# nicolaivicol/otto-recommender

Hardware: AMD Instinct MI355X
Metric: co-visit pairs/sec + candidates/sec at 220M events, 1/2/4/8 MI355X (higher is better)
Workload: dtype int32; 1 GPU; configs[1]: all 5 co-visitation rules, 220M events, 100k-session files; events=220000079, sessions=13435907, parallelism=files dealt over 1 GPU(s)

## Files before the change

### otto-recommender_amd/csrc/abi.hip

```cpp
#include <cstdarg>
#include <cstdlib>
#include <ctime>
#include <algorithm>
#include <mutex>
#include "prims.h"
#include "covis_kernels.h"
#include "table.h"

using namespace ottohip;

namespace ottohip {
static thread_local char g_err[1024] = "";
void set_error(const char* fmt, ...) {
  va_list ap;
  va_start(ap, fmt);
  vsnprintf(g_err, sizeof g_err, fmt, ap);
  va_end(ap);
}
}

namespace ottohip {
Ctx* ctx_base(ottohip_ctx* c) { return c; }

int ensure_part_stats(const ottohip_table* tc) {
// ... 566 lines not shown
  memset(&fo, 0, sizeof fo);
  if (fopts) OH_TRY(file_opts_setup(ctx, fopts, n_rules, R, fo, s));
  if (fo_parts) {
    fo = *fo_parts;
    OH_TRY(ctx->ws.get("fo_dropped", 1, &fo.dropped));
    OH_HIP(hipMemsetAsync(fo.dropped, 0, 8, s));
  }
  const bool FOon = fopts != nullptr || fo_parts != nullptr;
  const bool FOhist = FOon && !fo.cuts && !fo.parts && fo.hist != nullptr;
  const bool FOmir = FOon && fo.parts && fo.mirror_off != 0;
  const uint64_t n_slots = (fo_parts && fo_parts->mirror_off) ? 2 * P : P;
  if (ctx->spare.cap >= n_slots) {
    T->b = ctx->spare;
    ctx->spare = TableBufs();
  } else {
    const double t0 = alloc_log_begin();
    (void)hipDeviceSynchronize();
    ctx->spare.release();
    OH_TRY(T->b.alloc(n_slots));
    alloc_log_end(t0, "table", "slots", (size_t)n_slots * 17);
  }
  unsigned long long *stats, *lcount;
  OH_TRY(ws.get("stats", (size_t)STAT_STRIPES * STAT_STRIDE, &stats));
  OH_TRY(ws.get("lcount", 8, &lcount));
  hipMemsetAsync(stats, 0, (size_t)STAT_STRIPES * STAT_STRIDE * 8, s);
  hipMemsetAsync(err, 0, sizeof(int), s);
  if (getenv("OTTOHIP_REDUCE_DBG")) hipMemsetAsync(T->b.rule, 0xFF, n_slots, s);
  OutRows O;
  O.rule = T->b.rule; O.aid = T->b.aid; O.aid_next = T->b.aid_next; O.count = T->b.count; O.count_ge2 = T->b.count_ge2;
  O.cap = n_slots; O.stats = stats;
  T->sym_mask = R.sym_mask;
  static const int rdbg = getenv("OTTOHIP_REDUCE_DBG") ? atoi(getenv("OTTOHIP_REDUCE_DBG")) : 0;
  OutRows Osort = O;
  if (rdbg & 1) Osort.cap = 0;
  int herr = 0;

  static const int split_mean = getenv("OTTOHIP_SPLIT_MEAN") ? atoi(getenv("OTTOHIP_SPLIT_MEAN")) : SPLIT_MEAN;
  if (split_mean != SPLIT_MEAN) {
    const uint32_t v = (uint32_t)std::max(64, split_mean);
    OH_HIP(hipMemcpyToSymbolAsync(HIP_SYMBOL(c_split_mean), &v, sizeof v, 0, hipMemcpyHostToDevice, s));
    OH_HIP(hipStreamSynchronize(s));
  }
  static const char* runs_env = getenv("OTTOHIP_SPLIT_RUNS");
  if (runs_env && !strcmp(runs_env, "1")) {
    const uint32_t v = 1;
    OH_HIP(hipMemcpyToSymbolAsync(HIP_SYMBOL(c_split_runs), &v, sizeof v, 0, hipMemcpyHostToDevice, s));
    OH_HIP(hipStreamSynchronize(s));
// ... 10 lines not shown
    int8_t& st = lds_state[ctx->device & 63];
    if (st != (lds_leaf ? 2 : 1)) {
      const uint32_t on = lds_leaf ? 1u : 0u;
      OH_HIP(hipMemcpyToSymbolAsync(HIP_SYMBOL(c_lds_leaf), &on, sizeof on, 0, hipMemcpyHostToDevice, s));
      if (split_mean == SPLIT_MEAN) {
        const uint32_t v = lds_leaf ? (uint32_t)LDS_SPLIT_MEAN : (uint32_t)SPLIT_MEAN;
        OH_HIP(hipMemcpyToSymbolAsync(HIP_SYMBOL(c_split_mean), &v, sizeof v, 0, hipMemcpyHostToDevice, s));
      }
      OH_HIP(hipStreamSynchronize(s));
      st = lds_leaf ? 2 : 1;
    }
  }
  static const int hash_prio = getenv("OTTOHIP_HASH_PRIO") ? atoi(getenv("OTTOHIP_HASH_PRIO")) : 0;
  if (hash_prio) {
    const uint32_t v = (uint32_t)hash_prio;
    OH_HIP(hipMemcpyToSymbolAsync(HIP_SYMBOL(c_hash_prio), &v, sizeof v, 0, hipMemcpyHostToDevice, s));
    OH_HIP(hipStreamSynchronize(s));
  }
  int ph = ctx->begin("reduce", s, 4.0 * (double)P);
  uint64_t cap0 = (uint64_t)std::max<int64_t>(Rn, 1);
  TaskLists TL;
  TL.n = lcount;
  const uint64_t split_extra = P / 512 + 64;
  auto get_lists = [&](uint64_t capl, const char* split_name, int parity) -> int {
    static const char* names[2][N_SORT] = {{"t_sort0", "t_sort1", "t_sort2", "t_sort3", "t_sort4"},
                                           {"t_sort0b", "t_sort1b", "t_sort2b", "t_sort3b", "t_sort4b"}};
    for (int c = 0; c < N_SORT; ++c)
      if (int r = ws.get(names[parity][c], capl * sizeof(Task), reinterpret_cast<void**>(&TL.sort[c]))) return r;
    if (int r = ws.get(parity ? "t_hashb" : "t_hash", capl * sizeof(Task), reinterpret_cast<void**>(&TL.hash))) return r;
    if (int r = ws.get(parity ? "t_ldsb" : "t_lds", capl * sizeof(Task), reinterpret_cast<void**>(&TL.lds))) return r;
    if (int r = ws.get(split_name, (capl + split_extra) * sizeof(Task), reinterpret_cast<void**>(&TL.split))) return r;
    TL.cap = capl;
    return 0;
  };
  if ((rc = get_lists(cap0, "t_splitA", 0))) return rc;
  hipMemsetAsync(lcount, 0, 8 * 8, s);
  k_classify_rows<<<grid_for(Rn), 256, 0, s>>>(row_begin, Rn, P, Lt.WB, TL, err, row_base);
  const int agg_grid = ctx->n_cu * 8;
  static const bool overlap = !(getenv("OTTOHIP_REDUCE_OVERLAP") && !strcmp(getenv("OTTOHIP_REDUCE_OVERLAP"), "0"));
  hipStream_t s2 = nullptr;
  if (overlap) {
    OH_TRY(ctx->aux_stream());
    s2 = ctx->aux;
  }
  bool srcA = true;
  bool drained = false;
  const bool dbg = getenv("OTTOHIP_DEBUG") != nullptr;
  if (dbg) fprintf(stderr, "[ottohip] P=%llu rows=%lld\n", (unsigned long long)P, (long long)Rn);
  uint32_t* wcur0 = w0;
  const char* pipe_env = getenv("OTTOHIP_SPLIT_PIPE");
  const bool pipe = s2 != nullptr && !lds_leaf && !dbg && getenv("OTTOHIP_HASH_PROF") == nullptr &&
                    (pipe_env && atoi(pipe_env) == 1);
  const uint64_t PIPE_MIN_CHUNKS = getenv("OTTOHIP_SPLIT_PIPE_MIN") ? (uint64_t)atoll(getenv("OTTOHIP_SPLIT_PIPE_MIN")) : 2048;
  unsigned long long done[N_LISTS] = {};
  bool hash_early = false;
  auto launch_hash_range = [&](uint64_t lo, uint64_t hi, uint32_t* wb0, hipStream_t st) {
    if (hi <= lo) return;
    const int64_t nh = (int64_t)(hi - lo);
    const Task* th = TL.hash + lo;
    const unsigned hg = (unsigned)std::min<int64_t>(nh, (int64_t)agg_grid);
    if (FOhist)
      k_agg_hash<2><<<hg, AGG_T, 0, st>>>(th, nh, wb0, w1, row_key, R, Lt, n_rules, O, TL.split, lcount + N_SORT + 1, fo);
    else if (FOmir)
      k_agg_hash<3><<<hg, AGG_T, 0, st>>>(th, nh, wb0, w1, row_key, R, Lt, n_rules, O, TL.split, lcount + N_SORT + 1, fo);
    else if (FOon)
      k_agg_hash<1><<<hg, AGG_T, 0, st>>>(th, nh, wb0, w1, row_key, R, Lt, n_rules, O, TL.split, lcount + N_SORT + 1, fo);
    else
      k_agg_hash<<<hg, AGG_T, 0, st>>>(th, nh, wb0, w1, row_key, R, Lt, n_rules, O, TL.split, lcount + N_SORT + 1, fo);
  };
  auto launch_sorts = [&](const unsigned long long* lo, const unsigned long long* hi, uint32_t* wb0, hipStream_t st) {
    const unsigned sgrid = (unsigned)ctx->n_cu * 32;
#define OH_SORT(c, M)                                                                                          \
    if (hi[c] > lo[c]) {                                                                                       \
      const int64_t n_ = (int64_t)(hi[c] - lo[c]);                                                             \
      const Task* t_ = TL.sort[c] + lo[c];                                                                     \
      const unsigned g_ = (unsigned)std::min<uint64_t>(ceil_div(n_, 4), sgrid);                                \
      if (FOhist)                                                                                              \
        k_agg_sort<M, 2><<<g_, 256, (size_t)fo.nf * 8, st>>>(t_, n_, wb0, w1, row_key, R, Lt, n_rules, Osort, fo); \
      else if (FOmir)                                                                                          \
        k_agg_sort<M, 3><<<g_, 256, 0, st>>>(t_, n_, wb0, w1, row_key, R, Lt, n_rules, Osort, fo);             \
      else if (FOon)                                                                                           \
        k_agg_sort<M, 1><<<g_, 256, 0, st>>>(t_, n_, wb0, w1, row_key, R, Lt, n_rules, Osort, fo);             \
      else                                                                                                     \
        k_agg_sort<M><<<g_, 256, 0, st>>>(t_, n_, wb0, w1, row_key, R, Lt, n_rules, Osort, fo);                \
    }
    OH_SORT(0, 1) OH_SORT(1, 2) OH_SORT(2, 4) OH_SORT(3, 8) OH_SORT(4, 16)
#undef OH_SORT
  };
  for (int level = 0; level < 40; ++level) {
    wcur0 = (level == 0 || !w2) ? w0 : w2;
    unsigned long long nlist[N_LISTS];
    if ((rc = d2h(nlist, lcount, N_LISTS, s))) return rc;
    if ((rc = d2h(&herr, err, 1, s))) return rc;
    if (herr) { set_error("task list overflow / row too large (err=%d)", herr); return OTTOHIP_ELIMIT; }
    if (dbg) {
      fprintf(stderr, "[ottohip] level %d: sort %llu/%llu/%llu/%llu/%llu hash %llu split %llu lds %llu\n", level, nlist[0],
              nlist[1], nlist[2], nlist[3], nlist[4], nlist[N_SORT], nlist[N_SORT + 1], nlist[N_SORT + 2]);
      Task* lists[N_LISTS] = {TL.sort[0], TL.sort[1], TL.sort[2], TL.sort[3], TL.sort[4], TL.hash, TL.split, TL.lds};
      fprintf(stderr, "[ottohip] level %d words:", level);
      for (int c = 0; c < N_LISTS; ++c) {
        std::vector<Task> tv(nlist[c]);
        if (nlist[c]) (void)d2h(tv.data(), lists[c], nlist[c], s);
        unsigned long long sw = 0, mx = 0;
        for (auto& t : tv) { sw += t.len; mx = std::max<unsigned long long>(mx, t.len); }
        fprintf(stderr, " %llu(max %llu)", sw, mx);
        if (c == N_SORT + 1 && !tv.empty()) {
          unsigned long long hw[40] = {}, hn[40] = {};
          for (auto& t : tv) { const int b = 63 - __builtin_clzll((unsigned long long)t.len | 1ull); hw[b] += t.len; ++hn[b]; }
          fprintf(stderr, " [split by log2 len:");
          for (int b = 0; b < 40; ++b)
            if (hn[b]) fprintf(stderr, " 2^%d:%llu tasks/%llu words", b, hn[b], hw[b]);
          fprintf(stderr, "]");
        }
      }
      fprintf(stderr, "\n");
    }
    hipStream_t ss = s2 ? s2 : s;
    if (s2) { OH_HIP(hipEventRecord(ctx->ev_fork, s)); OH_HIP(hipStreamWaitEvent(s2, ctx->ev_fork, 0)); }
    static const bool hash_first = !(getenv("OTTOHIP_HASH_FIRST") && !strcmp(getenv("OTTOHIP_HASH_FIRST"), "0"));
    const bool hf = hash_first && nlist[N_SORT] > done[N_SORT];
    auto launch_hash = [&]() { launch_hash_range(done[N_SORT], nlist[N_SORT], wcur0, s); };
    if (hf) launch_hash();
    launch_sorts(done, nlist, wcur0, ss);
    if (s2) OH_HIP(hipEventRecord(ctx->ev_join[level & 1], s2));
    if (nlist[N_SORT + 2]) {
      const unsigned lg = (unsigned)std::min<uint64_t>(nlist[N_SORT + 2], (uint64_t)ctx->n_cu * 4);
      if (FOon)
        k_agg_lds<true><<<lg, LDS_T, 0, s>>>(TL.lds, (int64_t)nlist[N_SORT + 2], wcur0, w1, row_key, R, Lt, O, TL.split,
                                             lcount + N_SORT + 1, TL.cap + split_extra, err, fo);
      else
        k_agg_lds<<<lg, LDS_T, 0, s>>>(TL.lds, (int64_t)nlist[N_SORT + 2], wcur0, w1, row_key, R, Lt, O, TL.split,
                                       lcount + N_SORT + 1, TL.cap + split_extra, err, fo);
    }
    if (nlist[N_SORT] > done[N_SORT]) {
      static const bool hprof = getenv("OTTOHIP_HASH_PROF") != nullptr && !hash_first;
      if (hprof) {
        if ((rc = ws.get("hash_prof", (size_t)(2 * nlist[N_SORT]), &fo.prof))) return rc;
        OH_HIP(hipMemsetAsync(fo.prof, 0, 16 * nlist[N_SORT], s));
      }
      if (!hf) launch_hash();
      if (hprof) {
        std::vector<unsigned long long> pv(2 * nlist[N_SORT]);
        if ((rc = d2h(pv.data(), fo.prof, pv.size(), s))) return rc;
        std::vector<size_t> ord(nlist[N_SORT]);
// ... 32 lines not shown
        (rc = ws.get("sp_dgb", (size_t)ns + 1, &dgb)) || (rc = ws.get("sp_mtb", (size_t)ns + 1, &mtb)) ||
        (rc = ws.get("sp_tot", 6, &tot2)))
      return rc;
    k_split_prepare<<<grid_for(ns), 256, 0, s>>>(cur_split, ns, nch, ndg, nen);
    if ((rc = exclusive_scan_u32(ctx, nch, chb, ns, tot2, s)) || (rc = exclusive_scan_u32(ctx, ndg, dgb, ns, tot2 + 1, s)) ||
        (rc = exclusive_scan_u32(ctx, nen, mtb, ns, tot2 + 2, s)))
      return rc;
    if (pipe) k_split_half<<<1, 64, 0, s>>>(chb, dgb, ns, tot2, tot2 + 3);
    uint64_t tt[6] = {0, 0, 0, 0, 0, 0};
    if ((rc = d2h(tt, tot2, pipe ? 6 : 3, s))) return rc;
    const int64_t nchunks = (int64_t)tt[0], ndig = (int64_t)tt[1], nent = (int64_t)tt[2];
    const bool piped = pipe && (uint64_t)nchunks >= PIPE_MIN_CHUNKS && tt[3] > 0 && (int64_t)tt[3] < ns &&
                       tt[4] > 0 && (int64_t)tt[4] < nchunks && tt[5] > 0 && (int64_t)tt[5] < ndig;
    const uint32_t cA = piped ? (uint32_t)tt[4] : (uint32_t)nchunks;
    const int64_t dA = piped ? (int64_t)tt[5] : ndig;
    uint32_t *hmat, *ctask;
    uint64_t* hoff;
    if ((rc = ws.get("sp_hmat", (size_t)nent, &hmat)) || (rc = ws.get("sp_hoff", (size_t)nent + 1, &hoff)) ||
        (rc = ws.get("sp_ctask", (size_t)nchunks, &ctask)))
      return rc;
    k_split_chunk_task<<<grid_for(ns), 256, 0, s>>>(chb, nch, ns, ctask);
    k_split_hist<<<(unsigned)nchunks, SPLIT_T, 0, s>>>(cur_split, ns, chb, ctask, mtb, wcur0, w1, Lt.F, hmat);
    if ((rc = exclusive_scan_u32(ctx, hmat, hoff, nent, hoff + nent, s))) return rc;
    static const int sub = getenv("OTTOHIP_SPLIT_SUB") ? atoi(getenv("OTTOHIP_SPLIT_SUB")) : 4096;
    const char* lds_env = getenv("OTTOHIP_SPLIT_LDS");
    const bool split_lds = lds_env ? atoi(lds_env) != 0 : SPLIT_LDS_DEFAULT;
    const char* ldsmin_env = getenv("OTTOHIP_SPLIT_LDS_MIN");
    const uint32_t lds_min = (uint32_t)std::min(SPLIT_CH + 1, std::max(0, ldsmin_env ? atoi(ldsmin_env) : SPLIT_LDS_MIN));
    const int lds_t = getenv("OTTOHIP_SPLIT_LDS_T") ? atoi(getenv("OTTOHIP_SPLIT_LDS_T")) : SPLIT_LT;
    auto scatter = [&](uint32_t c0, uint32_t c1) {
      if (c1 <= c0) return;
      uint32_t max_len = SPLIT_CH;
      if (split_lds) {
        if (lds_t == 512)
          k_split_scatter_lds<512><<<c1 - c0, 512, 0, s>>>(cur_split, ns, chb, ctask, mtb, hoff, wcur0, w1, Lt.F, hmat, c0, lds_min);
        else
          k_split_scatter_lds<SPLIT_LT><<<c1 - c0, SPLIT_LT, 0, s>>>(cur_split, ns, chb, ctask, mtb, hoff, wcur0, w1, Lt.F, hmat, c0, lds_min);
        if (lds_min <= 1) return;
        max_len = lds_min - 1;
      }
      if (sub == 8192)
        k_split_scatter<8192><<<c1 - c0, SPLIT_T, 0, s>>>(cur_split, ns, chb, ctask, mtb, hoff, wcur0, w1, Lt.F, hmat, c0, max_len);
      else
        k_split_scatter<4096><<<c1 - c0, SPLIT_T, 0, s>>>(cur_split, ns, chb, ctask, mtb, hoff, wcur0, w1, Lt.F, hmat, c0, max_len);
    };
    scatter(0, cA);
    if (s2 && level >= 1) OH_HIP(hipStreamWaitEvent(s, ctx->ev_join[(level + 1) & 1], 0));
    const uint64_t capn = (uint64_t)ndig;
    if ((rc = get_lists(std::max(cap0, capn), srcA ? "t_splitB" : "t_splitA", (level + 1) & 1))) return rc;
    hipMemsetAsync(lcount, 0, 8 * 8, s);
    k_split_classify<<<grid_for(dA), 256, 0, s>>>(cur_split, ns, dgb, mtb, hoff, dA, TL, err, hmat, 0);
    if (piped) {
      if (getenv("OTTOHIP_SPLIT_PIPE_LOG")) fprintf(stderr, "[ottohip] level %d split pipelined at chunk %u of %lld\n", level, cA, (long long)nchunks);
      OH_HIP(hipEventRecord(ctx->ev_half, s));
      scatter(cA, (uint32_t)nchunks);
      if (ndig > dA)
        k_split_classify<<<grid_for(ndig - dA), 256, 0, s>>>(cur_split, ns, dgb, mtb, hoff, ndig, TL, err, hmat, dA);
      OH_HIP(hipStreamWaitEvent(ctx->aux2, ctx->ev_half, 0));
      unsigned long long nA[N_LISTS];
      if ((rc = d2h(nA, lcount, N_LISTS, ctx->aux2))) return rc;
      OH_HIP(hipStreamWaitEvent(s2, ctx->ev_half, 0));
      uint32_t* wb0 = w2 ? w2 : w0;
      if (nA[N_SORT]) {
        launch_hash_range(0, nA[N_SORT], wb0, s2);
        OH_HIP(hipEventRecord(ctx->ev_hash, s2));
        hash_early = true;
      }
      const unsigned long long zero[N_LISTS] = {};
      launch_sorts(zero, nA, wb0, s2);
      for (int c = 0; c <= N_SORT; ++c) done[c] = nA[c];
    }
    srcA = !srcA;
    if (hipGetLastError() != hipSuccess) { set_error("split launch failed"); return OTTOHIP_EHIP; }
  }
  ctx->end(ph, s);
  if (!drained) { set_error("reduce: split levels did not converge"); return OTTOHIP_ELIMIT; }
  std::vector<unsigned long long> stv((size_t)STAT_STRIPES * STAT_STRIDE);
  if ((rc = d2h(stv.data(), stats, stv.size(), s))) return rc;
  unsigned long long st[STAT_STRIDE] = {};
  for (int k = 0; k < STAT_STRIPES; ++k)
    for (int j = 0; j < STAT_STRIDE; ++j) st[j] += stv[(size_t)k * STAT_STRIDE + j];
  if (hipGetLastError() != hipSuccess) { set_error("reduce failed"); return OTTOHIP_EHIP; }
  unsigned long long U = 0, dropped = 0;
  for (int r = 0; r < n_rules; ++r) U += st[r * 4 + 0];
  const unsigned long long sum_pairs = st[STAT_RAW + 1], raw_rows = st[STAT_RAW];
  if (FOon) {
    if ((rc = d2h(&dropped, fo.dropped, 1, s))) return rc;
// ... 37 lines not shown
  if (hipHostMalloc(reinterpret_cast<void**>(&c->pinned), 64 * sizeof(uint64_t)) != hipSuccess) c->pinned = nullptr;
  *out = c;
  return 0;
}

void ottohip_ctx_destroy(ottohip_ctx* ctx) {
  if (!ctx) return;
  hipSetDevice(ctx->device);
  hipDeviceSynchronize();
  ctx->ws.release();
  ctx->spare.release();
  dev_trim();
  if (ctx->aux) {
    hipStreamDestroy(ctx->aux);
    if (ctx->aux2) hipStreamDestroy(ctx->aux2);
    if (ctx->ev_half) hipEventDestroy(ctx->ev_half);
    if (ctx->ev_hash) hipEventDestroy(ctx->ev_hash);
    hipEventDestroy(ctx->ev_fork);
    hipEventDestroy(ctx->ev_join[0]);
    hipEventDestroy(ctx->ev_join[1]);
  }
  for (auto e : ctx->event_pool) hipEventDestroy(e);
  if (ctx->pinned) hipHostFree(ctx->pinned);
  delete ctx;
}

int ottohip_ctx_trim(ottohip_ctx* ctx) {
  if (!ctx) return OTTOHIP_EINVAL;
  OH_HIP(hipSetDevice(ctx->device));
  OH_HIP(hipDeviceSynchronize());
  ctx->ws.release();
  ctx->spare.release();
  dev_trim();
  ctx->km_bvalid = false;
  ctx->km_hX = nullptr;
  ctx->om_items = -1;
  return 0;
}

int ottohip_ctx_set_timing(ottohip_ctx* ctx, int enable) {
  if (!ctx) return OTTOHIP_EINVAL;
  ctx->timing = enable != 0;
  return 0;
}

int ottohip_ctx_timing(ottohip_ctx* ctx, int idx, const char** name, float* ms, double* bytes) {
// ... 1022 lines not shown
```

### otto-recommender_amd/csrc/common.h

```cpp
#pragma once
#include <hip/hip_runtime.h>
#include <cstdint>
#include <cstdio>
#include <cstring>
#include <string>
#include <vector>
#include <map>
#include <type_traits>

#include "ottohip.h"

namespace ottohip {

constexpr int MAX_RULES = 8;

void set_error(const char* fmt, ...);
struct Ctx;
Ctx* ctx_base(ottohip_ctx* c);

#define OH_HIP(expr)                                                              \
  do {                                                                            \
    hipError_t e_ = (expr);                                                       \
    if (e_ != hipSuccess) {                                                       \
      ::ottohip::set_error("%s:%d %s -> %s", __FILE__, __LINE__, #expr,           \
                           hipGetErrorString(e_));                                \
      return e_ == hipErrorOutOfMemory ? OTTOHIP_ENOMEM : OTTOHIP_EHIP;           \
// ... 42 lines not shown
    auto it = bufs.find(name);
    if (it == bufs.end()) return nullptr;
    void* p = it->second.p;
    bufs.erase(it);
    return p;
  }
};

struct Phase { std::string name; hipEvent_t a, b; double bytes; };

struct Ctx {
  int device = 0;
  int n_cu = 256;
  Workspace ws;
  uint64_t* pinned = nullptr;
  bool timing = false;
  std::vector<Phase> phases;
  std::vector<hipEvent_t> event_pool;
  size_t event_used = 0;
  hipStream_t aux = nullptr;
  hipEvent_t ev_fork = nullptr, ev_join[2] = {nullptr, nullptr};
  hipStream_t aux2 = nullptr;
  hipEvent_t ev_half = nullptr, ev_hash = nullptr;
  int aux_stream() {
    if (aux) return 0;
    if (hipStreamCreateWithFlags(&aux, hipStreamNonBlocking) != hipSuccess ||
        hipStreamCreateWithFlags(&aux2, hipStreamNonBlocking) != hipSuccess ||
        hipEventCreateWithFlags(&ev_half, hipEventDisableTiming) != hipSuccess ||
        hipEventCreateWithFlags(&ev_hash, hipEventDisableTiming) != hipSuccess ||
        hipEventCreateWithFlags(&ev_fork, hipEventDisableTiming) != hipSuccess ||
        hipEventCreateWithFlags(&ev_join[0], hipEventDisableTiming) != hipSuccess ||
        hipEventCreateWithFlags(&ev_join[1], hipEventDisableTiming) != hipSuccess) {
      set_error("aux stream creation failed");
      return OTTOHIP_EHIP;
    }
    return 0;
  }
  hipEvent_t take_event() {
    if (event_used == event_pool.size()) {
      hipEvent_t e; hipEventCreate(&e); event_pool.push_back(e);
    }
    return event_pool[event_used++];
  }
  void reset_timing() { phases.clear(); event_used = 0; }
  int begin(const char* name, hipStream_t s, double bytes = 0) {
    if (!timing) return -1;
    Phase p; p.name = name; p.a = take_event(); p.b = take_event(); p.bytes = bytes;
    hipEventRecord(p.a, s);
    phases.push_back(p);
    return (int)phases.size() - 1;
// ... 133 lines not shown
```

### otto-recommender_amd/csrc/covis_kernels.h

```cpp
#pragma once
#include "prims.h"

namespace ottohip {

constexpr int EV_BLOCK = 256;
constexpr int LCAP = 512;
constexpr int SPLIT_MEAN = 420;
constexpr int LDS_SPLIT_MEAN = 2560;
__constant__ uint32_t c_split_mean = SPLIT_MEAN;
__constant__ uint32_t c_split_runs = 0;
__constant__ uint32_t c_split_fuse = 1;
__constant__ uint32_t c_hash_prio = 0;
__constant__ uint32_t c_lds_leaf = 0;
constexpr uint32_t W_EMPTY = 0xFFFFFFFFu;
constexpr int STAT_STRIPES = 256;
constexpr int STAT_RAW = MAX_RULES * 4;
constexpr int STAT_STRIDE = STAT_RAW + 8;

struct RulesDev {
  int32_t lo[MAX_RULES], hi[MAX_RULES];
  uint32_t mask[MAX_RULES];
  int32_t n_of_type[4];
  int32_t rule_of_type[4][MAX_RULES];
  uint32_t sym_mask;
// ... 2015 lines not shown
      } else if (k == W_EMPTY) {
        const unsigned long long nv = ((unsigned long long)key[j] << 32) | inc[j];
        if (atomicCAS(&slots[h[j]], v[j], nv) == v[j]) { slot[j] = h[j]; pend[j] = false; ++created; }
      } else {
        h[j] = (h[j] + 1) & cm;
        if (++probes[j] > cm) pend[j] = false;
      }
    }
  }
  return created;
}

constexpr int N_SORT = 5;
constexpr int SORT_MAX = 64 << (N_SORT - 1);
constexpr int LDS_CAP = 4096;
struct TaskLists {
  Task* sort[N_SORT];
  Task* hash;
  Task* split;
  Task* lds;
  unsigned long long* n;
  uint64_t cap;
};

template <int FOM = 0>
__global__ __launch_bounds__(AGG_T, 2) void k_agg_hash(const Task* __restrict__ tasks, int64_t n_tasks,
                                                    const uint32_t* __restrict__ w0, const uint32_t* __restrict__ w1,
                                                    const uint32_t* __restrict__ row_key, RulesDev R, Layout L,
                                                    int n_rules, OutRows O, Task* __restrict__ overflow,
                                                    unsigned long long* __restrict__ n_overflow, FileOpts fo) {
  __shared__ unsigned long long lds[2 * HCAP];
  __shared__ uint32_t wtot[AGG_T / 64];
  __shared__ uint32_t nocc;
  constexpr bool FO = FOM != 0, PM = FOM == 1 || FOM == 3;
  __shared__ unsigned long long fh[FO ? FO_MAXF : 1];
  __shared__ std::conditional_t<PM, PartLds, char> sP[1];
  const int tid = threadIdx.x;
  if (c_hash_prio == 1) __builtin_amdgcn_s_setprio(1);
  else if (c_hash_prio >= 2) __builtin_amdgcn_s_setprio(3);
  RuleAcc acc;
  acc.zero();
  if constexpr (FO) {
    for (uint32_t i = tid; i < fo.nf; i += AGG_T) fh[i] = 0;
    if constexpr (PM) part_lds_load(fo, sP[0]);
    __syncthreads();
  }
  const bool pmode = PM && fo.parts;
  for (int64_t ti = blockIdx.x; ti < n_tasks; ti += gridDim.x) {
    const Task T = tasks[ti];
    const uint64_t t_start = fo.prof ? wall_clock64() : 0;
    const uint32_t* W = (T.buf ? w1 : w0) + T.begin;
    const RowInfo ri = row_info(row_key, T.row, L.A);
    const bool fo_row = FO && ri.type == fo.type;
    const bool fo_cut = fo_row && (fo.cuts || fo.qonly);
    uint32_t ndrop = 0, dbg_loaded = 0, dbg_ins = 0;
    const uint32_t dbound = T.len;
    const bool optimistic = 2 * dbound > (uint32_t)HCAP;
    uint32_t cap = 64;
    while (cap < 2 * dbound && cap < (uint32_t)HCAP) cap <<= 1;
    const uint32_t cm = cap - 1, limit = (uint32_t)HCAP / 4;
    unsigned long long* A = lds;
    for (uint32_t i = tid; i < cap; i += AGG_T) A[i] = SLOT_EMPTY;
    if (tid == 0) nocc = 0;
    __syncthreads();
    bool full = false;
    constexpr int PF = 8;
    uint32_t wbuf[PF], nbuf[PF];
    const uint32_t l64 = (uint32_t)tid & 63u;
#pragma unroll
    for (int j = 0; j < PF; ++j) {
      const uint32_t i = j * AGG_T + tid;
// ... 27 lines not shown
        const uint64_t hm = __ballot(head);
        const uint64_t after = l64 == 63u ? 0ull : hm & (~0ull << (l64 + 1u));
        const uint32_t end = after ? (uint32_t)__builtin_ctzll(after) : 64u;
        inc[j] = end - l64;
        wbuf[j] = head ? w : W_EMPTY;
      }
      const uint32_t created = hash_insert_batch<PF>(A, wbuf, inc, cm, slot);
      if (FO && fo.dbg) {
#pragma unroll
        for (int j = 0; j < PF; ++j) dbg_ins += (wbuf[j] != W_EMPTY && slot[j] != HASH_FULL) ? inc[j] : 0u;
      }
#pragma unroll
      for (int j = 0; j < PF; ++j) full |= wbuf[j] != W_EMPTY && slot[j] == HASH_FULL;
      if (optimistic) {
        const uint32_t nc = wave_sum(created);
        if (nc && (tid & 63) == 0) atomicAdd(&nocc, nc);
      }
    }
    full = __syncthreads_or(full);
    if (full) {
      if (tid == 0) {
        const unsigned long long k = atomicAdd(n_overflow, 1ull);
        overflow[k] = T;
        if (fo.prof) {
          fo.prof[2 * ti] = T.len;
          fo.prof[2 * ti + 1] = (wall_clock64() - t_start) | (1ull << 63);
        }
      }
      __syncthreads();
      continue;
    }
    constexpr int SL = HCAP / AGG_T;
    uint32_t kw[SL], kc[SL];
#pragma unroll
    for (int s = 0; s < SL; ++s) {
      const uint32_t slot = tid + s * AGG_T;
      const unsigned long long v = slot < cap ? A[slot] : SLOT_EMPTY;
      kw[s] = (uint32_t)(v >> 32);
      kc[s] = (uint32_t)v;
    }
    if constexpr (FO) {
      const uint32_t nd = wave_sum(ndrop);
      if (nd && (tid & 63) == 0) atomicAdd(fo.dropped, (unsigned long long)nd);
      if (fo.dbg) {
        uint32_t kept = 0;
#pragma unroll
// ... 86 lines not shown
    if (fo.prof && tid == 0) {
      fo.prof[2 * ti] = T.len | ((unsigned long long)nout << 32);
      fo.prof[2 * ti + 1] = wall_clock64() - t_start;
    }
  }
  acc.flush(O.stats, n_rules);
  if constexpr (FO) {
    if (fo.hist) {
      __syncthreads();
      for (uint32_t i = tid; i < fo.nf; i += AGG_T)
        if (fh[i]) atomicAdd(&fo.hist[i], fh[i]);
    }
  }
}


constexpr int SPLIT_LEVELS = 4;
__device__ __forceinline__ int task_class(uint64_t len, uint32_t level, bool split) {
  for (int c = 0; c < N_SORT; ++c)
    if (len <= (uint64_t)(64 << c)) return c;
  if (split && c_lds_leaf && len <= (uint64_t)LDS_CAP && level < (uint32_t)SPLIT_LEVELS) return N_SORT + 2;
  return (split && level < (uint32_t)SPLIT_LEVELS) ? N_SORT + 1 : N_SORT;
}
constexpr int N_LISTS = N_SORT + 3;
__device__ __forceinline__ void push_task_block(const TaskLists& TL, bool valid, uint64_t begin, uint64_t len,
                                                uint32_t row, uint32_t rem, uint32_t buf, bool split, int* err) {
  __shared__ uint32_t bcnt[N_LISTS];
  __shared__ unsigned long long bbase[N_LISTS];
  if (valid && len > 0xFFFFFFFFull) { atomicOr(err, 2); valid = false; }
  const int c = valid ? task_class(len, rem, split) : -1;
  if (threadIdx.x < N_LISTS) bcnt[threadIdx.x] = 0;
  __syncthreads();
  uint32_t my = 0;
#pragma unroll
  for (int q = 0; q < N_LISTS; ++q) {
    const uint64_t m = __ballot(c == q);
    if (!m) continue;
    uint32_t wb = 0;
    if (mbcnt(m) == 0 && c == q) wb = atomicAdd(&bcnt[q], (uint32_t)__popcll(m));
    wb = __shfl(wb, __ffsll((long long)m) - 1);
    if (c == q) my = wb + mbcnt(m);
  }
  __syncthreads();
  if (threadIdx.x < N_LISTS && bcnt[threadIdx.x])
    bbase[threadIdx.x] = atomicAdd(&TL.n[threadIdx.x], (unsigned long long)bcnt[threadIdx.x]);
  __syncthreads();
  if (c >= 0) {
    const unsigned long long k = bbase[c] + my;
    Task t; t.begin = begin; t.len = (uint32_t)len; t.row = row; t.rem = rem; t.buf = buf;
    Task* list = c < N_SORT ? TL.sort[c] : (c == N_SORT ? TL.hash : (c == N_SORT + 1 ? TL.split : TL.lds));
    if (k < TL.cap) list[k] = t; else atomicOr(err, 4);
  }
}

__global__ void k_classify_rows(const uint64_t* __restrict__ row_begin, int64_t R, uint64_t P, int WB,
                                TaskLists TL, int* err, uint64_t row_base) {
  const int64_t r = (int64_t)blockIdx.x * blockDim.x + threadIdx.x;
  const bool valid = r < R;
  uint64_t b = 0, e = 0;
  if (valid) { b = row_begin[r] - row_base; e = r + 1 < R ? row_begin[r + 1] - row_base : P; }
  push_task_block(TL, valid && e > b, b, e - b, (uint32_t)r, 0u, 0u, true, err);
}

constexpr int SPLIT_CH = 16384;
__global__ void k_split_half(const uint64_t* __restrict__ chunk_base, const uint64_t* __restrict__ digit_base, int64_t n,
                             const uint64_t* __restrict__ nchunks_total, uint64_t* __restrict__ out) {
  if (threadIdx.x != 0 || blockIdx.x != 0) return;
  const uint64_t half = *nchunks_total / 2;
  int64_t lo = 0, hi = n;
  while (lo < hi) {
    const int64_t m = (lo + hi) >> 1;
    if (chunk_base[m] < half) lo = m + 1; else hi = m;
  }
  out[0] = (uint64_t)lo;
  out[1] = lo < n ? chunk_base[lo] : *nchunks_total;
  out[2] = lo < n ? digit_base[lo] : 0ull;
}
constexpr int SPLIT_T = 256;

constexpr int SPLIT_DMAX = 512;
__device__ __forceinline__ uint32_t split_ndig(const Task& t) {
  const uint64_t d = ((uint64_t)t.len + c_split_mean - 1) / c_split_mean;
  return d < 2 ? 2u : (d > (uint64_t)SPLIT_DMAX ? (uint32_t)SPLIT_DMAX : (uint32_t)d);
}
__device__ __forceinline__ uint32_t split_digit(uint32_t w, int F, uint32_t level, uint32_t nd) {
  uint32_t x = (w >> F) ^ (level * 0x9E3779B9u);
  x ^= x >> 16; x *= 0x7feb352du; x ^= x >> 15; x *= 0x846ca68bu; x ^= x >> 16;
  return (uint32_t)(((uint64_t)x * nd) >> 32);
}
__global__ void k_split_prepare(const Task* __restrict__ tasks, int64_t n, uint32_t* __restrict__ nchunks,
                                uint32_t* __restrict__ ndigits, uint32_t* __restrict__ nent) {
  const int64_t i = (int64_t)blockIdx.x * blockDim.x + threadIdx.x;
  if (i >= n) return;
  const uint32_t nch = (uint32_t)ceil_div((int64_t)tasks[i].len, SPLIT_CH), nd = split_ndig(tasks[i]);
  nchunks[i] = nch;
  ndigits[i] = nd;
  nent[i] = nch * nd;
}

__device__ __forceinline__ int64_t find_task(const uint64_t* chunk_base, int64_t n, uint64_t c) {
  int64_t lo = 0, hi = n;
  while (hi - lo > 1) {
    const int64_t m = (lo + hi) >> 1;
    if (chunk_base[m] <= c) lo = m; else hi = m;
  }
  return lo;
}
// ... 1125 lines not shown
```

Baseline: 85.08 billion pairs/s.

## Add scheduled reduce levels with precomputed split work and dynamic hash task queue

Adds an opt-in reduce scheduler that counts split chunk, digit and entry totals during classification. It reads all level counters in one pinned copy and runs the hash kernel on a third stream, so hash overflow feeds the next level instead of serializing. By default, hash launches now use an occupancy-sized persistent grid that pulls tasks from an atomic counter, replacing the fixed strided grid, and aux streams get priorities. The cost is extra atomics in classification and in per-task hash dispatch, plus added synchronization inside the hash block loop.

```diff
diff --git a/otto-recommender_amd/csrc/abi.hip b/otto-recommender_amd/csrc/abi.hip
--- a/otto-recommender_amd/csrc/abi.hip
+++ b/otto-recommender_amd/csrc/abi.hip
@@ -612,7 +612,7 @@
   }
   unsigned long long *stats, *lcount;
   OH_TRY(ws.get("stats", (size_t)STAT_STRIPES * STAT_STRIDE, &stats));
-  OH_TRY(ws.get("lcount", 8, &lcount));
+  OH_TRY(ws.get("lcount", 2 * LC_WORDS, &lcount));
   hipMemsetAsync(stats, 0, (size_t)STAT_STRIPES * STAT_STRIDE * 8, s);
   hipMemsetAsync(err, 0, sizeof(int), s);
   if (getenv("OTTOHIP_REDUCE_DBG")) hipMemsetAsync(T->b.rule, 0xFF, n_slots, s);
@@ -669,20 +669,18 @@
   TaskLists TL;
   TL.n = lcount;
   const uint64_t split_extra = P / 512 + 64;
-  auto get_lists = [&](uint64_t capl, const char* split_name, int parity) -> int {
+  auto get_lists = [&](uint64_t capl, const char* split_name, int parity, uint64_t more_split = 0) -> int {
     static const char* names[2][N_SORT] = {{"t_sort0", "t_sort1", "t_sort2", "t_sort3", "t_sort4"},
                                            {"t_sort0b", "t_sort1b", "t_sort2b", "t_sort3b", "t_sort4b"}};
     for (int c = 0; c < N_SORT; ++c)
       if (int r = ws.get(names[parity][c], capl * sizeof(Task), reinterpret_cast<void**>(&TL.sort[c]))) return r;
     if (int r = ws.get(parity ? "t_hashb" : "t_hash", capl * sizeof(Task), reinterpret_cast<void**>(&TL.hash))) return r;
     if (int r = ws.get(parity ? "t_ldsb" : "t_lds", capl * sizeof(Task), reinterpret_cast<void**>(&TL.lds))) return r;
-    if (int r = ws.get(split_name, (capl + split_extra) * sizeof(Task), reinterpret_cast<void**>(&TL.split))) return r;
+    if (int r = ws.get(split_name, (capl + split_extra + more_split) * sizeof(Task), reinterpret_cast<void**>(&TL.split))) return r;
     TL.cap = capl;
     return 0;
   };
   if ((rc = get_lists(cap0, "t_splitA", 0))) return rc;
-  hipMemsetAsync(lcount, 0, 8 * 8, s);
-  k_classify_rows<<<grid_for(Rn), 256, 0, s>>>(row_begin, Rn, P, Lt.WB, TL, err, row_base);
   const int agg_grid = ctx->n_cu * 8;
   static const bool overlap = !(getenv("OTTOHIP_REDUCE_OVERLAP") && !strcmp(getenv("OTTOHIP_REDUCE_OVERLAP"), "0"));
   hipStream_t s2 = nullptr;
@@ -690,30 +688,54 @@
     OH_TRY(ctx->aux_stream());
     s2 = ctx->aux;
   }
+  const char* pipe_env = getenv("OTTOHIP_SPLIT_PIPE");
+  const bool pipe_on = pipe_env && atoi(pipe_env) == 1;
+  const char* sched_env = getenv("OTTOHIP_REDUCE_SCHED");
+  const bool sched = s2 != nullptr && sched_env && atoi(sched_env) == 1 && !pipe_on && !lds_leaf &&
+                     getenv("OTTOHIP_HASH_PROF") == nullptr;
+  auto level_err = [&](int set) { return sched ? reinterpret_cast<int*>(lcount + set * LC_WORDS + LC_ERR) : err; };
+  hipMemsetAsync(lcount, 0, 2 * LC_WORDS * 8, s);
+  k_classify_rows<<<grid_for(Rn), 256, 0, s>>>(row_begin, Rn, P, Lt.WB, TL, level_err(0), row_base);
+  const char* hgrid_env = getenv("OTTOHIP_HASH_GRID");
+  const int hgrid = hgrid_env ? std::max(0, atoi(hgrid_env)) : -1;
+  const int fom = FOhist ? 2 : (FOmir ? 3 : (FOon ? 1 : 0));
+  unsigned int* hnext = nullptr;
+  if (hgrid != 0) OH_TRY(ws.get("hash_next", 2, &hnext));
+  if (hgrid < 0 && !ctx->hash_resident[fom]) {
+    int nb = 0;
+    hipError_t e = fom == 2   ? hipOccupancyMaxActiveBlocksPerMultiprocessor(&nb, k_agg_hash<2>, AGG_T, 0)
+                   : fom == 3 ? hipOccupancyMaxActiveBlocksPerMultiprocessor(&nb, k_agg_hash<3>, AGG_T, 0)
+                   : fom == 1 ? hipOccupancyMaxActiveBlocksPerMultiprocessor(&nb, k_agg_hash<1>, AGG_T, 0)
+                              : hipOccupancyMaxActiveBlocksPerMultiprocessor(&nb, k_agg_hash<0>, AGG_T, 0);
+    if (e != hipSuccess || nb < 1) { set_error("k_agg_hash<%d>: occupancy query failed", fom); return OTTOHIP_EHIP; }
+    ctx->hash_resident[fom] = nb * ctx->n_cu;
+  }
   bool srcA = true;
   bool drained = false;
   const bool dbg = getenv("OTTOHIP_DEBUG") != nullptr;
   if (dbg) fprintf(stderr, "[ottohip] P=%llu rows=%lld\n", (unsigned long long)P, (long long)Rn);
   uint32_t* wcur0 = w0;
-  const char* pipe_env = getenv("OTTOHIP_SPLIT_PIPE");
-  const bool pipe = s2 != nullptr && !lds_leaf && !dbg && getenv("OTTOHIP_HASH_PROF") == nullptr &&
-                    (pipe_env && atoi(pipe_env) == 1);
+  const bool pipe = s2 != nullptr && !lds_leaf && !dbg && getenv("OTTOHIP_HASH_PROF") == nullptr && pipe_on;
   const uint64_t PIPE_MIN_CHUNKS = getenv("OTTOHIP_SPLIT_PIPE_MIN") ? (uint64_t)atoll(getenv("OTTOHIP_SPLIT_PIPE_MIN")) : 2048;
   unsigned long long done[N_LISTS] = {};
   bool hash_early = false;
-  auto launch_hash_range = [&](uint64_t lo, uint64_t hi, uint32_t* wb0, hipStream_t st) {
+  auto launch_hash_range = [&](uint64_t lo, uint64_t hi, uint32_t* wb0, hipStream_t st, Task* ov,
+                               unsigned long long* n_ov, unsigned long long* ov_work, int slot) {
     if (hi <= lo) return;
     const int64_t nh = (int64_t)(hi - lo);
     const Task* th = TL.hash + lo;
-    const unsigned hg = (unsigned)std::min<int64_t>(nh, (int64_t)agg_grid);
+    const int64_t blocks = hgrid == 0 ? (int64_t)agg_grid : (hgrid > 0 ? (int64_t)hgrid : (int64_t)ctx->hash_resident[fom]);
+    const unsigned hg = (unsigned)std::min<int64_t>(nh, blocks);
+    unsigned int* nt = hgrid == 0 ? nullptr : hnext + slot;
+    if (nt) hipMemsetAsync(nt, 0, sizeof(unsigned int), st);
     if (FOhist)
-      k_agg_hash<2><<<hg, AGG_T, 0, st>>>(th, nh, wb0, w1, row_key, R, Lt, n_rules, O, TL.split, lcount + N_SORT + 1, fo);
+      k_agg_hash<2><<<hg, AGG_T, 0, st>>>(th, nh, wb0, w1, row_key, R, Lt, n_rules, O, ov, n_ov, fo, nt, ov_work);
     else if (FOmir)
-      k_agg_hash<3><<<hg, AGG_T, 0, st>>>(th, nh, wb0, w1, row_key, R, Lt, n_rules, O, TL.split, lcount + N_SORT + 1, fo);
+      k_agg_hash<3><<<hg, AGG_T, 0, st>>>(th, nh, wb0, w1, row_key, R, Lt, n_rules, O, ov, n_ov, fo, nt, ov_work);
     else if (FOon)
-      k_agg_hash<1><<<hg, AGG_T, 0, st>>>(th, nh, wb0, w1, row_key, R, Lt, n_rules, O, TL.split, lcount + N_SORT + 1, fo);
+      k_agg_hash<1><<<hg, AGG_T, 0, st>>>(th, nh, wb0, w1, row_key, R, Lt, n_rules, O, ov, n_ov, fo, nt, ov_work);
     else
-      k_agg_hash<<<hg, AGG_T, 0, st>>>(th, nh, wb0, w1, row_key, R, Lt, n_rules, O, TL.split, lcount + N_SORT + 1, fo);
+      k_agg_hash<<<hg, AGG_T, 0, st>>>(th, nh, wb0, w1, row_key, R, Lt, n_rules, O, ov, n_ov, fo, nt, ov_work);
   };
   auto launch_sorts = [&](const unsigned long long* lo, const unsigned long long* hi, uint32_t* wb0, hipStream_t st) {
     const unsigned sgrid = (unsigned)ctx->n_cu * 32;
@@ -734,7 +756,109 @@
     OH_SORT(0, 1) OH_SORT(1, 2) OH_SORT(2, 4) OH_SORT(3, 8) OH_SORT(4, 16)
 #undef OH_SORT
   };
-  for (int level = 0; level < 40; ++level) {
+  static const int sub = getenv("OTTOHIP_SPLIT_SUB") ? atoi(getenv("OTTOHIP_SPLIT_SUB")) : 4096;
+  const char* lds_env = getenv("OTTOHIP_SPLIT_LDS");
+  const bool split_lds = lds_env ? atoi(lds_env) != 0 : SPLIT_LDS_DEFAULT;
+  const char* ldsmin_env = getenv("OTTOHIP_SPLIT_LDS_MIN");
+  const uint32_t lds_min = (uint32_t)std::min(SPLIT_CH + 1, std::max(0, ldsmin_env ? atoi(ldsmin_env) : SPLIT_LDS_MIN));
+  const int lds_t = getenv("OTTOHIP_SPLIT_LDS_T") ? atoi(getenv("OTTOHIP_SPLIT_LDS_T")) : SPLIT_LT;
+  auto scatter_chunks = [&](const Task* cur_split, int64_t ns, const uint64_t* chb, const uint32_t* ctask, const uint64_t* mtb,
+                            const uint64_t* hoff, uint32_t* hmat, uint32_t c0, uint32_t c1) {
+    if (c1 <= c0) return;
+    uint32_t max_len = SPLIT_CH;
+    if (split_lds) {
+      if (lds_t == 512)
+        k_split_scatter_lds<512><<<c1 - c0, 512, 0, s>>>(cur_split, ns, chb, ctask, mtb, hoff, wcur0, w1, Lt.F, hmat, c0, lds_min);
+      else
+        k_split_scatter_lds<SPLIT_LT><<<c1 - c0, SPLIT_LT, 0, s>>>(cur_split, ns, chb, ctask, mtb, hoff, wcur0, w1, Lt.F, hmat, c0, lds_min);
+      if (lds_min <= 1) return;
+      max_len = lds_min - 1;
+    }
+    if (sub == 8192)
+      k_split_scatter<8192><<<c1 - c0, SPLIT_T, 0, s>>>(cur_split, ns, chb, ctask, mtb, hoff, wcur0, w1, Lt.F, hmat, c0, max_len);
+    else
+      k_split_scatter<4096><<<c1 - c0, SPLIT_T, 0, s>>>(cur_split, ns, chb, ctask, mtb, hoff, wcur0, w1, Lt.F, hmat, c0, max_len);
+  };
+  auto sched_levels = [&]() -> int {
+    OH_TRY(ctx->level_buffer());
+    hipStream_t s3 = ctx->aux2;
+    const unsigned long long* hv = ctx->level_host;
+    Task* ovl[2] = {nullptr, nullptr};
+    bool hash_pending = false;
+    for (int level = 0; level < 40; ++level) {
+      const int p = level & 1;
+      unsigned long long* C = lcount + p * LC_WORDS;
+      unsigned long long* Cn = lcount + (p ^ 1) * LC_WORDS;
+      wcur0 = (level == 0 || !w2) ? w0 : w2;
+      if (hash_pending) OH_HIP(hipStreamWaitEvent(s, ctx->ev_hash, 0));
+      hash_pending = false;
+      OH_HIP(hipMemcpyAsync(ctx->level_host, C, LC_WORDS * 8, hipMemcpyDeviceToHost, s));
+      OH_HIP(hipMemsetAsync(Cn, 0, LC_WORDS * 8, s));
+      OH_HIP(hipEventRecord(ctx->ev_fork, s));
+      OH_HIP(hipStreamSynchronize(s));
+      if (hv[LC_ERR]) {
+        set_error("task list overflow / row too large (err=%d)", (int)hv[LC_ERR]);
+        return OTTOHIP_ELIMIT;
+      }
+      unsigned long long nlist[N_LISTS];
+      for (int c = 0; c < N_LISTS; ++c) nlist[c] = hv[c];
+      const uint64_t nh = nlist[N_SORT], nov = hv[LC_OVERFLOW];
+      const int64_t nsl = (int64_t)nlist[N_SORT + 1], ns = nsl + (int64_t)nov;
+      const int64_t nchunks = (int64_t)hv[LC_CHUNKS], ndig = (int64_t)hv[LC_DIGITS], nent = (int64_t)hv[LC_ENTRIES];
+      if (dbg)
+        fprintf(stderr, "[ottohip] level %d: sort %llu/%llu/%llu/%llu/%llu hash %llu split %llu lds %llu overflow %llu "
+                "(chunks %lld digits %lld entries %lld)\n", level, nlist[0], nlist[1], nlist[2], nlist[3], nlist[4],
+                (unsigned long long)nh, nlist[N_SORT + 1], nlist[N_SORT + 2], (unsigned long long)nov, (long long)nchunks,
+                (long long)ndig, (long long)nent);
+      if ((uint64_t)nsl > TL.cap) { set_error("split list overflow"); return OTTOHIP_ELIMIT; }
+      if (nh) {
+        if ((rc = ws.get(p ? "t_overB" : "t_overA", (size_t)nh, &ovl[p]))) return rc;
+        OH_HIP(hipStreamWaitEvent(s3, ctx->ev_fork, 0));
+        launch_hash_range(0, nh, wcur0, s3, ovl[p], Cn + LC_OVERFLOW, Cn + LC_CHUNKS, 0);
+        OH_HIP(hipEventRecord(ctx->ev_hash, s3));
+        hash_pending = true;
+      }
+      OH_HIP(hipStreamWaitEvent(s2, ctx->ev_fork, 0));
+      const unsigned long long zero[N_LISTS] = {};
+      launch_sorts(zero, nlist, wcur0, s2);
+      OH_HIP(hipEventRecord(ctx->ev_join[p], s2));
+      if (ns == 0 && !hash_pending) {
+        OH_HIP(hipStreamWaitEvent(s, ctx->ev_join[p], 0));
+        drained = true;
+        return 0;
+      }
+      Task* cur_split = TL.split;
+      uint32_t *nch, *ndg, *nen, *hmat = nullptr;
+      uint64_t *chb, *dgb = nullptr, *mtb = nullptr, *tot2, *hoff = nullptr;
+      if (ns) {
+        if (nov)
+          OH_HIP(hipMemcpyAsync(cur_split + nsl, ovl[p ^ 1], (size_t)nov * sizeof(Task), hipMemcpyDeviceToDevice, s));
+        uint32_t* ctask;
+        if ((rc = ws.get("sp_nch", (size_t)ns, &nch)) || (rc = ws.get("sp_ndg", (size_t)ns, &ndg)) ||
+            (rc = ws.get("sp_nen", (size_t)ns, &nen)) || (rc = ws.get("sp_chb", (size_t)ns + 1, &chb)) ||
+            (rc = ws.get("sp_dgb", (size_t)ns + 1, &dgb)) || (rc = ws.get("sp_mtb", (size_t)ns + 1, &mtb)) ||
+            (rc = ws.get("sp_tot", 6, &tot2)) || (rc = ws.get("sp_hmat", (size_t)nent, &hmat)) ||
+            (rc = ws.get("sp_hoff", (size_t)nent + 1, &hoff)) || (rc = ws.get("sp_ctask", (size_t)nchunks, &ctask)))
+          return rc;
+        k_split_prepare<<<grid_for(ns), 256, 0, s>>>(cur_split, ns, nch, ndg, nen);
+        if ((rc = exclusive_scan_u32(ctx, nch, chb, ns, tot2, s)) || (rc = exclusive_scan_u32(ctx, ndg, dgb, ns, tot2 + 1, s)) ||
+            (rc = exclusive_scan_u32(ctx, nen, mtb, ns, tot2 + 2, s)))
+          return rc;
+        k_split_chunk_task<<<grid_for(ns), 256, 0, s>>>(chb, nch, ns, ctask);
+        k_split_hist<<<(unsigned)nchunks, SPLIT_T, 0, s>>>(cur_split, ns, chb, ctask, mtb, wcur0, w1, Lt.F, hmat);
+        if ((rc = exclusive_scan_u32(ctx, hmat, hoff, nent, hoff + nent, s))) return rc;
+        scatter_chunks(cur_split, ns, chb, ctask, mtb, hoff, hmat, 0, (uint32_t)nchunks);
+      }
+      if (level >= 1) OH_HIP(hipStreamWaitEvent(s, ctx->ev_join[p ^ 1], 0));
+      if ((rc = get_lists(std::max(cap0, (uint64_t)ndig), p ? "t_splitA" : "t_splitB", p ^ 1, nh))) return rc;
+      TL.n = Cn;
+      if (ns) k_split_classify<<<grid_for(ndig), 256, 0, s>>>(cur_split, ns, dgb, mtb, hoff, ndig, TL, level_err(p ^ 1), hmat, 0);
+      if (hipGetLastError() != hipSuccess) { set_error("split launch failed"); return OTTOHIP_EHIP; }
+    }
+    return 0;
+  };
+  if (sched) OH_TRY(sched_levels());
+  for (int level = 0; !sched && level < 40; ++level) {
     wcur0 = (level == 0 || !w2) ? w0 : w2;
     unsigned long long nlist[N_LISTS];
     if ((rc = d2h(nlist, lcount, N_LISTS, s))) return rc;
@@ -766,7 +890,9 @@
     if (s2) { OH_HIP(hipEventRecord(ctx->ev_fork, s)); OH_HIP(hipStreamWaitEvent(s2, ctx->ev_fork, 0)); }
     static const bool hash_first = !(getenv("OTTOHIP_HASH_FIRST") && !strcmp(getenv("OTTOHIP_HASH_FIRST"), "0"));
     const bool hf = hash_first && nlist[N_SORT] > done[N_SORT];
-    auto launch_hash = [&]() { launch_hash_range(done[N_SORT], nlist[N_SORT], wcur0, s); };
+    auto launch_hash = [&]() {
+      launch_hash_range(done[N_SORT], nlist[N_SORT], wcur0, s, TL.split, lcount + N_SORT + 1, nullptr, 0);
+    };
     if (hf) launch_hash();
     launch_sorts(done, nlist, wcur0, ss);
     if (s2) OH_HIP(hipEventRecord(ctx->ev_join[level & 1], s2));
@@ -845,33 +971,12 @@
     k_split_chunk_task<<<grid_for(ns), 256, 0, s>>>(chb, nch, ns, ctask);
     k_split_hist<<<(unsigned)nchunks, SPLIT_T, 0, s>>>(cur_split, ns, chb, ctask, mtb, wcur0, w1, Lt.F, hmat);
     if ((rc = exclusive_scan_u32(ctx, hmat, hoff, nent, hoff + nent, s))) return rc;
-    static const int sub = getenv("OTTOHIP_SPLIT_SUB") ? atoi(getenv("OTTOHIP_SPLIT_SUB")) : 4096;
-    const char* lds_env = getenv("OTTOHIP_SPLIT_LDS");
-    const bool split_lds = lds_env ? atoi(lds_env) != 0 : SPLIT_LDS_DEFAULT;
-    const char* ldsmin_env = getenv("OTTOHIP_SPLIT_LDS_MIN");
-    const uint32_t lds_min = (uint32_t)std::min(SPLIT_CH + 1, std::max(0, ldsmin_env ? atoi(ldsmin_env) : SPLIT_LDS_MIN));
-    const int lds_t = getenv("OTTOHIP_SPLIT_LDS_T") ? atoi(getenv("OTTOHIP_SPLIT_LDS_T")) : SPLIT_LT;
-    auto scatter = [&](uint32_t c0, uint32_t c1) {
-      if (c1 <= c0) return;
-      uint32_t max_len = SPLIT_CH;
-      if (split_lds) {
-        if (lds_t == 512)
-          k_split_scatter_lds<512><<<c1 - c0, 512, 0, s>>>(cur_split, ns, chb, ctask, mtb, hoff, wcur0, w1, Lt.F, hmat, c0, lds_min);
-        else
-          k_split_scatter_lds<SPLIT_LT><<<c1 - c0, SPLIT_LT, 0, s>>>(cur_split, ns, chb, ctask, mtb, hoff, wcur0, w1, Lt.F, hmat, c0, lds_min);
-        if (lds_min <= 1) return;
-        max_len = lds_min - 1;
-      }
-      if (sub == 8192)
-        k_split_scatter<8192><<<c1 - c0, SPLIT_T, 0, s>>>(cur_split, ns, chb, ctask, mtb, hoff, wcur0, w1, Lt.F, hmat, c0, max_len);
-      else
-        k_split_scatter<4096><<<c1 - c0, SPLIT_T, 0, s>>>(cur_split, ns, chb, ctask, mtb, hoff, wcur0, w1, Lt.F, hmat, c0, max_len);
-    };
+    auto scatter = [&](uint32_t c0, uint32_t c1) { scatter_chunks(cur_split, ns, chb, ctask, mtb, hoff, hmat, c0, c1); };
     scatter(0, cA);
     if (s2 && level >= 1) OH_HIP(hipStreamWaitEvent(s, ctx->ev_join[(level + 1) & 1], 0));
     const uint64_t capn = (uint64_t)ndig;
     if ((rc = get_lists(std::max(cap0, capn), srcA ? "t_splitB" : "t_splitA", (level + 1) & 1))) return rc;
-    hipMemsetAsync(lcount, 0, 8 * 8, s);
+    hipMemsetAsync(lcount, 0, LC_WORDS * 8, s);
     k_split_classify<<<grid_for(dA), 256, 0, s>>>(cur_split, ns, dgb, mtb, hoff, dA, TL, err, hmat, 0);
     if (piped) {
       if (getenv("OTTOHIP_SPLIT_PIPE_LOG")) fprintf(stderr, "[ottohip] level %d split pipelined at chunk %u of %lld\n", level, cA, (long long)nchunks);
@@ -885,7 +990,7 @@
       OH_HIP(hipStreamWaitEvent(s2, ctx->ev_half, 0));
       uint32_t* wb0 = w2 ? w2 : w0;
       if (nA[N_SORT]) {
-        launch_hash_range(0, nA[N_SORT], wb0, s2);
+        launch_hash_range(0, nA[N_SORT], wb0, s2, TL.split, lcount + N_SORT + 1, nullptr, 1);
         OH_HIP(hipEventRecord(ctx->ev_hash, s2));
         hash_early = true;
       }
@@ -969,6 +1074,7 @@
   }
   for (auto e : ctx->event_pool) hipEventDestroy(e);
   if (ctx->pinned) hipHostFree(ctx->pinned);
+  if (ctx->level_host) hipHostFree(ctx->level_host);
   delete ctx;
 }
 
diff --git a/otto-recommender_amd/csrc/common.h b/otto-recommender_amd/csrc/common.h
--- a/otto-recommender_amd/csrc/common.h
+++ b/otto-recommender_amd/csrc/common.h
@@ -2,6 +2,7 @@
 #include <hip/hip_runtime.h>
 #include <cstdint>
 #include <cstdio>
+#include <cstdlib>
 #include <cstring>
 #include <string>
 #include <vector>
@@ -90,10 +91,24 @@
   hipEvent_t ev_fork = nullptr, ev_join[2] = {nullptr, nullptr};
   hipStream_t aux2 = nullptr;
   hipEvent_t ev_half = nullptr, ev_hash = nullptr;
+  unsigned long long* level_host = nullptr;
+  int hash_resident[4] = {0, 0, 0, 0};
+  int level_buffer() {
+    if (level_host) return 0;
+    if (hipHostMalloc(reinterpret_cast<void**>(&level_host), 32 * sizeof(unsigned long long)) != hipSuccess) {
+      level_host = nullptr;
+      set_error("pinned level buffer allocation failed");
+      return OTTOHIP_ENOMEM;
+    }
+    return 0;
+  }
   int aux_stream() {
     if (aux) return 0;
-    if (hipStreamCreateWithFlags(&aux, hipStreamNonBlocking) != hipSuccess ||
-        hipStreamCreateWithFlags(&aux2, hipStreamNonBlocking) != hipSuccess ||
+    const int prio = getenv("OTTOHIP_AUX_PRIO") ? atoi(getenv("OTTOHIP_AUX_PRIO")) : 1;
+    int least = 0, greatest = 0;
+    if (prio > 0 && hipDeviceGetStreamPriorityRange(&least, &greatest) != hipSuccess) least = greatest = 0;
+    if (hipStreamCreateWithPriority(&aux, hipStreamNonBlocking, prio > 0 ? least : 0) != hipSuccess ||
+        hipStreamCreateWithPriority(&aux2, hipStreamNonBlocking, prio > 1 ? greatest : 0) != hipSuccess ||
         hipEventCreateWithFlags(&ev_half, hipEventDisableTiming) != hipSuccess ||
         hipEventCreateWithFlags(&ev_hash, hipEventDisableTiming) != hipSuccess ||
         hipEventCreateWithFlags(&ev_fork, hipEventDisableTiming) != hipSuccess ||
diff --git a/otto-recommender_amd/csrc/covis_kernels.h b/otto-recommender_amd/csrc/covis_kernels.h
--- a/otto-recommender_amd/csrc/covis_kernels.h
+++ b/otto-recommender_amd/csrc/covis_kernels.h
@@ -2061,14 +2061,26 @@
   unsigned long long* n;
   uint64_t cap;
 };
+constexpr int N_LISTS = N_SORT + 3;
+constexpr int LC_CHUNKS = N_LISTS, LC_DIGITS = N_LISTS + 1, LC_ENTRIES = N_LISTS + 2, LC_OVERFLOW = N_LISTS + 3,
+              LC_ERR = N_LISTS + 4, LC_WORDS = 16;
+static_assert(LC_ERR < LC_WORDS, "counter set");
+__device__ __forceinline__ uint32_t split_ndig_len(uint64_t len);
+__device__ __forceinline__ void split_work(uint64_t len, uint32_t& nch, uint32_t& nd) {
+  nch = (uint32_t)((len + 16383ull) / 16384ull);
+  nd = split_ndig_len(len);
+}
 
 template <int FOM = 0>
 __global__ __launch_bounds__(AGG_T, 2) void k_agg_hash(const Task* __restrict__ tasks, int64_t n_tasks,
                                                     const uint32_t* __restrict__ w0, const uint32_t* __restrict__ w1,
                                                     const uint32_t* __restrict__ row_key, RulesDev R, Layout L,
                                                     int n_rules, OutRows O, Task* __restrict__ overflow,
-                                                    unsigned long long* __restrict__ n_overflow, FileOpts fo) {
+                                                    unsigned long long* __restrict__ n_overflow, FileOpts fo,
+                                                    unsigned int* __restrict__ next_task = nullptr,
+                                                    unsigned long long* __restrict__ ov_work = nullptr) {
   __shared__ unsigned long long lds[2 * HCAP];
+  __shared__ unsigned int s_next;
   __shared__ uint32_t wtot[AGG_T / 64];
   __shared__ uint32_t nocc;
   constexpr bool FO = FOM != 0, PM = FOM == 1 || FOM == 3;
@@ -2085,7 +2097,14 @@
     __syncthreads();
   }
   const bool pmode = PM && fo.parts;
-  for (int64_t ti = blockIdx.x; ti < n_tasks; ti += gridDim.x) {
+  auto take_task = [&](int64_t prev) -> int64_t {
+    if (!next_task) return prev < 0 ? (int64_t)blockIdx.x : prev + (int64_t)gridDim.x;
+    __syncthreads();
+    if (tid == 0) s_next = atomicAdd(next_task, 1u);
+    __syncthreads();
+    return (int64_t)s_next;
+  };
+  for (int64_t ti = take_task(-1); ti < n_tasks; ti = take_task(ti)) {
     const Task T = tasks[ti];
     const uint64_t t_start = fo.prof ? wall_clock64() : 0;
     const uint32_t* W = (T.buf ? w1 : w0) + T.begin;
@@ -2159,6 +2178,13 @@
       if (tid == 0) {
         const unsigned long long k = atomicAdd(n_overflow, 1ull);
         overflow[k] = T;
+        if (ov_work) {
+          uint32_t nch, nd;
+          split_work(T.len, nch, nd);
+          atomicAdd(ov_work + 0, (unsigned long long)nch);
+          atomicAdd(ov_work + 1, (unsigned long long)nd);
+          atomicAdd(ov_work + 2, (unsigned long long)nch * nd);
+        }
         if (fo.prof) {
           fo.prof[2 * ti] = T.len;
           fo.prof[2 * ti + 1] = (wall_clock64() - t_start) | (1ull << 63);
@@ -2291,14 +2317,15 @@
   if (split && c_lds_leaf && len <= (uint64_t)LDS_CAP && level < (uint32_t)SPLIT_LEVELS) return N_SORT + 2;
   return (split && level < (uint32_t)SPLIT_LEVELS) ? N_SORT + 1 : N_SORT;
 }
-constexpr int N_LISTS = N_SORT + 3;
 __device__ __forceinline__ void push_task_block(const TaskLists& TL, bool valid, uint64_t begin, uint64_t len,
                                                 uint32_t row, uint32_t rem, uint32_t buf, bool split, int* err) {
   __shared__ uint32_t bcnt[N_LISTS];
   __shared__ unsigned long long bbase[N_LISTS];
+  __shared__ unsigned long long bwork[3];
   if (valid && len > 0xFFFFFFFFull) { atomicOr(err, 2); valid = false; }
   const int c = valid ? task_class(len, rem, split) : -1;
   if (threadIdx.x < N_LISTS) bcnt[threadIdx.x] = 0;
+  if (threadIdx.x < 3) bwork[threadIdx.x] = 0;
   __syncthreads();
   uint32_t my = 0;
 #pragma unroll
@@ -2309,10 +2336,22 @@
     if (mbcnt(m) == 0 && c == q) wb = atomicAdd(&bcnt[q], (uint32_t)__popcll(m));
     wb = __shfl(wb, __ffsll((long long)m) - 1);
     if (c == q) my = wb + mbcnt(m);
+    if (q == N_SORT + 1) {
+      uint32_t nch = 0, nd = 0;
+      if (c == q) split_work(len, nch, nd);
+      const uint64_t s0 = wave_sum64(nch), s1 = wave_sum64(nd), s2 = wave_sum64((uint64_t)nch * nd);
+      if (lane_id() == 0) {
+        atomicAdd(&bwork[0], (unsigned long long)s0);
+        atomicAdd(&bwork[1], (unsigned long long)s1);
+        atomicAdd(&bwork[2], (unsigned long long)s2);
+      }
+    }
   }
   __syncthreads();
   if (threadIdx.x < N_LISTS && bcnt[threadIdx.x])
     bbase[threadIdx.x] = atomicAdd(&TL.n[threadIdx.x], (unsigned long long)bcnt[threadIdx.x]);
+  if (threadIdx.x >= 64 && threadIdx.x < 67 && bcnt[N_SORT + 1])
+    atomicAdd(&TL.n[LC_CHUNKS + threadIdx.x - 64], bwork[threadIdx.x - 64]);
   __syncthreads();
   if (c >= 0) {
     const unsigned long long k = bbase[c] + my;
@@ -2348,10 +2387,12 @@
 constexpr int SPLIT_T = 256;
 
 constexpr int SPLIT_DMAX = 512;
-__device__ __forceinline__ uint32_t split_ndig(const Task& t) {
-  const uint64_t d = ((uint64_t)t.len + c_split_mean - 1) / c_split_mean;
+__device__ __forceinline__ uint32_t split_ndig_len(uint64_t len) {
+  const uint64_t d = (len + c_split_mean - 1) / c_split_mean;
   return d < 2 ? 2u : (d > (uint64_t)SPLIT_DMAX ? (uint32_t)SPLIT_DMAX : (uint32_t)d);
 }
+__device__ __forceinline__ uint32_t split_ndig(const Task& t) { return split_ndig_len(t.len); }
+static_assert(SPLIT_CH == 16384, "split_work");
 __device__ __forceinline__ uint32_t split_digit(uint32_t w, int F, uint32_t level, uint32_t nd) {
   uint32_t x = (w >> F) ^ (level * 0x9E3779B9u);
   x ^= x >> 16; x *= 0x7feb352du; x ^= x >> 15; x *= 0x846ca68bu; x ^= x >> 16;
```

After: 87.20 billion pairs/s, median of 6. 1.02x the previous value.
